# knights-lab/UTree

Measured on NVIDIA B200. Metric: reads/sec (150bp, L2-scale CTR, RC); k-mer lookups/sec in lookups_per_s, higher is better.
Workload: dtype u64

## Files before the change

utree_b200/csrc/kernels.cu:

```cuda
#include <cuda_runtime.h>
#include <stdint.h>
#include <stdio.h>
#include <stdlib.h>
#include <string.h>
#include "utb_internal.h"

#define SUFMASK 0xFFFFFFFFFFull
#define HIT_MISS 0xFFFFFFFFu
#define HIT_NOWIN 0xFFFFFFFEu

#define CK(call)                                                                 \
    do {                                                                         \
        cudaError_t e_ = (call);                                                 \
        if (e_ != cudaSuccess) {                                                 \
            utb_set_error("CUDA error %s at %s:%d (%s)", cudaGetErrorName(e_),   \
                          __FILE__, __LINE__, cudaGetErrorString(e_));           \
            return UTB_ERR_CUDA;                                                 \
        }                                                                        \
    } while (0)

struct DevDB {
    const uint32_t *binix32;
    const uint64_t *binix64;
    const uint8_t *recs;
// ... 26 lines not shown
    int sm_count;
    size_t nb_binix, nb_recs, nb_blob, nb_lab, nb_ktab, nb_sieve;
    int l2_window;
    size_t l2_window_bytes;
    float l2_hit_ratio;
};

__device__ __forceinline__ uint32_t classify4(uint32_t w, uint32_t &badbits) {
    const uint32_t u = w | 0x20202020u;
    const uint32_t code = ((u >> 1) ^ (u >> 2)) & 0x03030303u;
    const uint32_t c0 = code & 0x01010101u, c1 = (code >> 1) & 0x01010101u;
    const uint32_t both = c0 & c1;
    const uint32_t expect = 0x61616161u + (((c0 | c1) << 1) | ((c1 & ~c0) << 2)) + both * 0x11u;
    const uint32_t x = u ^ expect;
    const uint32_t inval = ((((x & 0x7F7F7F7Fu) + 0x7F7F7F7Fu) | x) >> 7) & 0x01010101u;
    badbits = (inval * 0x01020408u) >> 24;
    return code;
}

__device__ __forceinline__ uint64_t revcomp_word(uint64_t w) {
    uint64_t x = __brevll(~w);
    return ((x >> 1) & 0x5555555555555555ull) | ((x & 0x5555555555555555ull) << 1);
}
__device__ __forceinline__ uint64_t word_to_planes(uint64_t w) {
    uint64_t t;
    t = (w ^ (w >> 1)) & 0x2222222222222222ull; w ^= t ^ (t << 1);
    t = (w ^ (w >> 2)) & 0x0C0C0C0C0C0C0C0Cull; w ^= t ^ (t << 2);
    t = (w ^ (w >> 4)) & 0x00F000F000F000F0ull; w ^= t ^ (t << 4);
    t = (w ^ (w >> 8)) & 0x0000FF000000FF00ull; w ^= t ^ (t << 8);
    t = (w ^ (w >> 16)) & 0x00000000FFFF0000ull; w ^= t ^ (t << 16);
    return w;
}
__device__ __forceinline__ uint64_t planes_to_word(uint64_t w) {
    uint64_t t;
    t = (w ^ (w >> 16)) & 0x00000000FFFF0000ull; w ^= t ^ (t << 16);
    t = (w ^ (w >> 8)) & 0x0000FF000000FF00ull; w ^= t ^ (t << 8);
    t = (w ^ (w >> 4)) & 0x00F000F000F000F0ull; w ^= t ^ (t << 4);
    t = (w ^ (w >> 2)) & 0x0C0C0C0C0C0C0C0Cull; w ^= t ^ (t << 2);
    t = (w ^ (w >> 1)) & 0x2222222222222222ull; w ^= t ^ (t << 1);
    return w;
}
__device__ __forceinline__ uint32_t group_read(const uint32_t *__restrict__ grp_off, uint32_t n_reads, uint32_t g0, uint32_t lane) {
    uint32_t lo = 0, hi = n_reads;
    while (hi - lo > 1) {
        uint32_t mid = (lo + hi) >> 1;
        if (__ldg(grp_off + mid) <= g0) lo = mid; else hi = mid;
    }
    const uint32_t nb = lo + 1u + lane;
    const uint32_t bnd = nb < n_reads ? __ldg(grp_off + nb) : 0xFFFFFFFFu;
    const uint32_t starts = __reduce_or_sync(0xFFFFFFFFu, bnd - g0 < 32u ? 1u << (bnd - g0) : 0u);
    return lo + __popc(starts & (0xFFFFFFFFu >> (31u - lane)));
}
#define PK_GUARD 8u
template <bool WORDS, bool PLANES>
__global__ void __launch_bounds__(256)
pack_kernel(const uint8_t *__restrict__ raw, const uint64_t *__restrict__ seq_off,
            const uint32_t *__restrict__ seq_len, const uint32_t *__restrict__ grp_off,
            uint32_t n_reads, uint32_t n_groups, const uint32_t *__restrict__ dims,
            uint64_t *__restrict__ pk, uint32_t *__restrict__ bad, uint64_t *__restrict__ pl, uint32_t *__restrict__ rid) {
    if (dims) { n_reads = dims[0]; n_groups = dims[1]; }
    const uint32_t lane = threadIdx.x & 31u;
    for (uint64_t gw = ((uint64_t)blockIdx.x * blockDim.x + threadIdx.x) & ~31ull; gw < (uint64_t)n_groups + PK_GUARD; gw += (uint64_t)gridDim.x * blockDim.x) {
        const uint32_t g = (uint32_t)gw + lane;
        const uint32_t lo = (uint32_t)gw < n_groups ? group_read(grp_off, n_reads, (uint32_t)gw, lane) : 0u;
        if (g >= n_groups + PK_GUARD) continue;
        if (g >= n_groups) {
            if (WORDS) pk[g] = 0;
            if (PLANES) pl[g] = 0;
            bad[g] = 0xFFFFFFFFu;
            continue;
        }
        uint32_t k = g - __ldg(grp_off + lo);
        uint32_t len = __ldg(seq_len + lo);
        if (rid) rid[g] = lo;
        uint32_t b0 = k * 32u;
        uint32_t nv = len > b0 ? min(32u, len - b0) : 0u;
        uint64_t word = 0;
        uint32_t p1 = 0, p0 = 0;
        uint32_t badm = 0;
        if (nv) {
            uint64_t a = __ldg(seq_off + lo) + b0;
            const uint32_t *p = reinterpret_cast<const uint32_t *>(raw + (a & ~3ull));
            uint32_t sh = (uint32_t)(a & 3u) * 8u;
            uint32_t nw = (nv + 3u) >> 2;
            uint32_t prev = __ldg(p);
#pragma unroll
            for (uint32_t j = 0; j < 8; ++j) {
                uint32_t cur = (j < nw) ? __ldg(p + j + 1) : 0u;
                uint32_t w = __funnelshift_r(prev, cur, sh);
                prev = cur;
                uint32_t bb;
                const uint32_t code = classify4(w, bb);
                if (WORDS) word = (word << 8) | ((code * 0x40100401u) >> 24);
                if (PLANES) {
                    p1 = (p1 << 4) | ((((code >> 1) & 0x01010101u) * 0x08040201u) >> 24);
                    p0 = (p0 << 4) | (((code & 0x01010101u) * 0x08040201u) >> 24);
                }
                badm |= bb << (4u * j);
            }
        }
        if (nv < 32u) badm |= 0xFFFFFFFFu << nv;
        if (WORDS) pk[g] = word;
        if (PLANES) pl[g] = ((uint64_t)p1 << 32) | p0;
        bad[g] = badm;
    }
}

__device__ __forceinline__ bool window_at(const uint64_t *__restrict__ pk, const uint32_t *__restrict__ bad,
                                          uint32_t pos, uint64_t &w) {
    uint32_t g = pos >> 5, o = pos & 31u;
    uint64_t hi = pk[g], lo = pk[g + 1];
    uint32_t bh = bad[g], bl = bad[g + 1];
    uint32_t wb = o ? ((bh >> o) | (bl << (32u - o))) : bh;
    w = o ? ((hi << (2u * o)) | (lo >> (64u - 2u * o))) : hi;
    return wb == 0;
}


__device__ __forceinline__ uint64_t load_suffix(const uint8_t *__restrict__ recs, uint64_t byte_addr) {
    const uint32_t *p = reinterpret_cast<const uint32_t *>(recs + (byte_addr & ~3ull));
    uint32_t w0 = __ldg(p), w1 = __ldg(p + 1);
    uint32_t sh = (uint32_t)(byte_addr & 3u) * 8u;
    uint64_t v = ((uint64_t)w1 << 32) | w0;
    return (v >> sh) & SUFMASK;
}

__device__ __forceinline__ uint32_t load_ix(const DevDB &db, uint64_t rec) {
    const uint8_t *r = db.recs + rec * db.sz + 5;
    uint32_t v = (uint32_t)__ldg(r) | ((uint32_t)__ldg(r + 1) << 8);
    if (db.ix_bytes == 4) v |= ((uint32_t)__ldg(r + 2) << 16) | ((uint32_t)__ldg(r + 3) << 24);
    return v;
}

struct Probe {
    uint64_t pos, size, suf;
    bool live;
};

__device__ __forceinline__ void probe_begin(const DevDB &db, uint64_t word, Probe &q) {
    uint64_t p = word >> 40;
    uint64_t a, b;
    if (db.binix32) { a = __ldg(db.binix32 + p); b = __ldg(db.binix32 + p + 1); }
    else { a = __ldg(db.binix64 + p); b = __ldg(db.binix64 + p + 1); }
    q.suf = word & SUFMASK;
    q.live = a < b;
    if (b > db.num_nodes) q.live = false;
    q.pos = a;
    q.size = q.live ? b - a - 1 : 0;
}

template <int N>
__device__ __forceinline__ void probe_run(const DevDB &db, Probe (&q)[N]) {
    for (;;) {
        bool any = false;
#pragma unroll
        for (int i = 0; i < N; ++i) any |= q[i].size != 0;
// ... 223 lines not shown
    uint32_t r = HIT_NOWIN, ns = 0;
    if (valid) {
        if (NSTR == 2 && (slot & 1)) w = revcomp_word(w);
        if (TABLE) r = kt_lookup(db, w, &ns);
        else {
            Probe q[1];
            probe_begin(db, w, q[0]);
            probe_run<1>(db, q);
            r = probe_end(db, q[0]);
        }
    }
    if (pos < n_pos) hits[slot] = r;
    const uint32_t nv = __popc(__ballot_sync(0xFFFFFFFFu, valid));
    const uint32_t nh = __popc(__ballot_sync(0xFFFFFFFFu, r < HIT_NOWIN));
    for (int o = 16; o; o >>= 1) ns += __shfl_xor_sync(0xFFFFFFFFu, ns, o);
    if ((threadIdx.x & 31u) == 0) {
        const uint32_t c = blockIdx.x & (COUNTER_SLOTS - 1);
        if (nv) atomicAdd(counters + c, (unsigned long long)nv);
        if (nh) atomicAdd(counters + COUNTER_SLOTS + c, (unsigned long long)nh);
        if (ns) atomicAdd(counters + 3 * COUNTER_SLOTS + c, (unsigned long long)ns);
    }
}

#define Q_CHUNK 128u
#define Q_INVALID 0xFFFFFFFFu
struct WarpQueue {
    uint64_t base;
    uint32_t used;
    bool have;
};
__device__ __forceinline__ void wq_init(WarpQueue &q) { q.base = 0; q.used = Q_CHUNK; q.have = false; }
__device__ __forceinline__ void wq_retire(const WarpQueue &q, uint32_t lane, uint32_t *__restrict__ q_slots) {
    if (q.have) for (uint32_t j = q.used + lane; j < Q_CHUNK; j += 32) q_slots[q.base + j] = Q_INVALID;
}
__device__ __forceinline__ void wq_reserve(WarpQueue &q, uint32_t c, uint32_t lane, uint32_t *__restrict__ q_slots,
                                           unsigned long long *__restrict__ q_count, uint64_t q_cap) {
    if (q.used + c <= Q_CHUNK) return;
    wq_retire(q, lane, q_slots);
    unsigned long long nb = 0;
    if (lane == 0) nb = atomicAdd(q_count, (unsigned long long)Q_CHUNK);
    q.base = __shfl_sync(0xFFFFFFFFu, nb, 0);
    q.used = 0;
    q.have = q.base + Q_CHUNK <= q_cap;
}
struct HitSink {
    uint32_t *hits;
    uint32_t *hitmap;
    const uint32_t *rid, *grp_off;
    uint32_t *cnt;
    uint32_t sh;
};
__device__ __forceinline__ void sink_put(const HitSink &k, uint32_t slot, uint32_t r) {
    if (k.cnt) {
        const uint32_t rd = __ldg(k.rid + (slot >> k.sh));
        k.hits[((uint64_t)__ldg(k.grp_off + rd) << k.sh) + atomicAdd(k.cnt + rd, 1u)] = r;
    } else { k.hits[slot] = r; atomicOr(k.hitmap + (slot >> 5), 1u << (slot & 31u)); }
}
__device__ __noinline__ uint32_t resolve_inline(const DevDB &db, uint64_t x, uint32_t slot, const HitSink &sink) {
    const uint32_t r = kt_lookup(db, planes_to_word(x));
    if (r == HIT_MISS) return 0;
    sink_put(sink, slot, r);
    return 1;
}
template <int NSTR>
__device__ __forceinline__ uint32_t emit_survivors(const DevDB &db, WarpQueue &wq, uint32_t lane, bool passF, bool passR, uint64_t w, uint64_t rc,
                                                   uint32_t pos, uint64_t *__restrict__ q_words, uint32_t *__restrict__ q_slots,
                                                   unsigned long long *__restrict__ q_count, uint64_t q_cap, const HitSink &sink) {
    const uint32_t bF = __ballot_sync(0xFFFFFFFFu, passF);
    const uint32_t bR = NSTR == 2 ? __ballot_sync(0xFFFFFFFFu, passR) : 0u;
    const uint32_t cF = __popc(bF), c = cF + __popc(bR);
    uint32_t nh = 0;
    if (!c) return 0;
    wq_reserve(wq, c, lane, q_slots, q_count, q_cap);
    const uint32_t lt = (1u << lane) - 1u;
    if (wq.have) {
        const uint64_t at = wq.base + wq.used;
        if (passF) { const uint64_t i = at + __popc(bF & lt); q_words[i] = w; q_slots[i] = pos * NSTR; }
        if (passR) { const uint64_t i = at + cF + __popc(bR & lt); q_words[i] = rc; q_slots[i] = pos * NSTR + 1u; }
    } else {
        if (passF) nh += resolve_inline(db, w, pos * NSTR, sink);
        if (passR) nh += resolve_inline(db, rc, pos * NSTR + 1u, sink);
    }
    wq.used += c;
    return nh;
}

#define SV_DEAD 0xFFFFFFFFu
struct SvStep { uint32_t w1, w0, h, blk; };
__device__ __forceinline__ void sv_step(uint64_t cur, uint64_t next, uint32_t bh, uint32_t bl, uint32_t lane, SvStep &s) {
    s.w1 = __funnelshift_l((uint32_t)(next >> 32), (uint32_t)(cur >> 32), lane);
    s.w0 = __funnelshift_l((uint32_t)next, (uint32_t)cur, lane);
    const uint32_t m = sv_kmer16(s.w1, s.w0);
    s.h = sv_mhash(m, sv_rc16(m));
    s.blk = __funnelshift_r(bh, bl, lane) == 0u ? 0u : SV_DEAD;
}
template <int D, int SV_U>
__device__ __forceinline__ void sv_shifted(const uint32_t (&x)[SV_U + 1], uint32_t (&y)[SV_U + 1], uint32_t lane) {
    uint32_t rot[SV_U + 1];
#pragma unroll
    for (int u = 0; u <= SV_U; ++u) rot[u] = __shfl_sync(0xFFFFFFFFu, x[u], (lane + D) & 31u);
    const bool same = lane + D < 32u;
#pragma unroll
    for (int u = 0; u < SV_U; ++u) y[u] = same ? rot[u] : rot[u + 1];
    y[SV_U] = rot[SV_U];
}
__device__ __forceinline__ void sv_prefetch(const void *p) { asm volatile("prefetch.global.L1 [%0];" ::"l"(p)); }
template <int NSTR, int SV_U, int SV_MINB>
__global__ void __launch_bounds__(256, SV_MINB)
sieve_kernel(DevDB db, const uint64_t *__restrict__ pl, const uint32_t *__restrict__ bad, uint32_t n_pos,
             const uint32_t *__restrict__ n_groups_dev, unsigned long long *__restrict__ counters,
             uint64_t *__restrict__ q_words, uint32_t *__restrict__ q_slots, unsigned long long *__restrict__ q_count,
             uint64_t q_cap, const HitSink sink) {
    if (n_groups_dev) n_pos = *n_groups_dev * 32u;
    const uint32_t lane = threadIdx.x & 31u;
    const uint32_t n_steps = n_pos >> 5;
    const uint32_t n_warps = gridDim.x * (blockDim.x >> 5), wid = blockIdx.x * (blockDim.x >> 5) + (threadIdx.x >> 5);
    uint32_t per = (n_steps + n_warps - 1) / n_warps;
    per = (per + SV_U - 1) / SV_U * SV_U;
    const uint64_t s0 = (uint64_t)wid * per;
    const uint32_t s1 = s0 + per < n_steps ? (uint32_t)(s0 + per) : n_steps;
    const uint2 *__restrict__ sieve = db.sieve;
    const uint32_t n_lines = db.sv_lines;
    WarpQueue wq;
    wq_init(wq);
    uint32_t nv = 0, nh = 0;
    if (s0 < s1) {
        SvStep st[SV_U + 1];
        uint64_t cur = __ldg(pl + s0), next = __ldg(pl + s0 + 1);
        uint32_t bh = __ldg(bad + s0), bl = __ldg(bad + s0 + 1);
        sv_step(cur, next, bh, bl, lane, st[0]);
        for (uint32_t s = (uint32_t)s0; s < s1; s += SV_U) {
            {
                const uint32_t pf = s + 32u < n_steps ? s + 32u : n_steps;
                sv_prefetch(pl + pf); sv_prefetch(bad + pf);
            }
#pragma unroll
            for (int u = 1; u <= SV_U; ++u) {
                cur = next; bh = bl;
                next = __ldg(pl + s + u + 1); bl = __ldg(bad + s + u + 1);
                sv_step(cur, next, bh, bl, lane, st[u]);
            }
            uint32_t x[SV_U + 1], y1[SV_U + 1], y2[SV_U + 1];
#pragma unroll
            for (int u = 0; u <= SV_U; ++u) x[u] = st[u].h;
            sv_shifted<16, SV_U>(x, y1, lane);
#pragma unroll
            for (int u = 0; u < SV_U; ++u) st[u].blk |= sv_block(x[u], y1[u]);
            sv_shifted<1, SV_U>(x, y1, lane); sv_shifted<2, SV_U>(x, y2, lane);
#pragma unroll
            for (int u = 0; u <= SV_U; ++u) x[u] = __vimin3_u32(x[u], y1[u], y2[u]);
            sv_shifted<3, SV_U>(x, y1, lane); sv_shifted<6, SV_U>(x, y2, lane);
#pragma unroll
            for (int u = 0; u <= SV_U; ++u) x[u] = __vimin3_u32(x[u], y1[u], y2[u]);
            sv_shifted<8, SV_U>(x, y1, lane);
#pragma unroll
            for (int u = 0; u < SV_U; ++u) x[u] = x[u] < y1[u] ? x[u] : y1[u];
            uint2 v[SV_U];
#pragma unroll
            for (int u = 0; u < SV_U; ++u) {
                v[u] = make_uint2(0, 0);
                if (st[u].blk != SV_DEAD) v[u] = __ldg(sieve + ((sv_line(x[u], n_lines) << 4) | st[u].blk));
            }
#pragma unroll
            for (int u = 0; u < SV_U; ++u) {
                const bool live = st[u].blk != SV_DEAD;
                if (__any_sync(0xFFFFFFFFu, live)) {
                    const uint32_t r1 = ~__brev(st[u].w1), r0 = ~__brev(st[u].w0);
                    const bool tF = sv_test(v[u], st[u].w1, st[u].w0), tR = NSTR == 2 && sv_test(v[u], r1, r0);
                    nh += emit_survivors<NSTR>(db, wq, lane, live & tF, live & tR, ((uint64_t)st[u].w1 << 32) | st[u].w0, ((uint64_t)r1 << 32) | r0,
                                               (s + u) * 32u + lane, q_words, q_slots, q_count, q_cap, sink);
                    nv += live ? NSTR : 0;
                }
            }
            st[0] = st[SV_U];
        }
    }
    wq_retire(wq, lane, q_slots);
    for (int o = 16; o; o >>= 1) { nv += __shfl_xor_sync(0xFFFFFFFFu, nv, o); nh += __shfl_xor_sync(0xFFFFFFFFu, nh, o); }
    if (lane == 0) {
        const uint32_t cs = (blockIdx.x * 8 + (threadIdx.x >> 5)) & (COUNTER_SLOTS - 1);
        if (nv) atomicAdd(counters + cs, (unsigned long long)nv);
        if (nh) atomicAdd(counters + COUNTER_SLOTS + cs, (unsigned long long)nh);
    }
}

template <bool LISTS>
__global__ void __launch_bounds__(256, 6)
queue_lookup_kernel(DevDB db, const uint64_t *__restrict__ q_words, const uint32_t *__restrict__ q_slots,
                    const unsigned long long *__restrict__ q_count, uint64_t q_cap,
                    const HitSink sink, unsigned long long *__restrict__ counters) {
    const uint64_t n = *q_count < q_cap ? *q_count : q_cap;
    const uint64_t stride = (uint64_t)gridDim.x * blockDim.x;
// ... 1559 lines not shown
    memset(vs, 0, sizeof *vs);
}
static int vs_alloc(const utb_db *db, size_t max_bytes, vote_scratch *vs) {
    memset(vs, 0, sizeof *vs);
    const size_t nl = db->d.max_ix ? db->d.max_ix : 1;
    vs->n_cta = (unsigned)db->sm_count * VB_PER_SM;
    size_t pool = ((size_t)384 << 20) / (12 * nl);
    if (pool > VBIG_POOL_MAX) pool = VBIG_POOL_MAX;
    if (pool < 1) pool = 1;
    vs->vl.pool = (uint32_t)pool;
    vs->vl.split_slots = (size_t)128 << 10;
    (void)max_bytes;
    const char *e = getenv("UTB_VOTE_SPLIT_SLOTS");
    if (e && atoll(e) > 0) vs->vl.split_slots = (unsigned long long)atoll(e);
    vs->vl.sort_max = VB_SORT_MAX;
    e = getenv("UTB_VOTE_SORT_MAX");
    if (e && atoi(e) >= 0 && (uint32_t)atoi(e) < VB_SORT_MAX) vs->vl.sort_max = (uint32_t)atoi(e);
    cudaError_t err = cudaMalloc(&vs->vl.hist, (size_t)vs->n_cta * nl * 4);
    if (err == cudaSuccess) err = cudaMalloc(&vs->vl.tlab, (size_t)vs->n_cta * nl * 4);
    if (err == cudaSuccess) err = cudaMalloc(&vs->vl.tcnt, (size_t)vs->n_cta * nl * 4);
    if (err == cudaSuccess) err = cudaMalloc(&vs->vl.big_hist, pool * nl * 4);
    if (err == cudaSuccess) err = cudaMalloc(&vs->vl.big_tlab, pool * nl * 4);
    if (err == cudaSuccess) err = cudaMalloc(&vs->vl.big_tcnt, pool * nl * 4);
    if (err == cudaSuccess) err = cudaMalloc(&vs->vl.big_list, pool * 4);
    if (err == cudaSuccess) err = cudaMalloc(&vs->vl.big_state, (1 + 2 * pool) * 4);
    if (err == cudaSuccess) err = cudaMalloc(&vs->vl.work, 4);
    if (err == cudaSuccess) err = cudaMemset(vs->vl.hist, 0, (size_t)vs->n_cta * nl * 4);
    if (err == cudaSuccess) err = cudaMemset(vs->vl.big_hist, 0, pool * nl * 4);
    if (err != cudaSuccess) { vs_free(vs); CK(err); }
    return UTB_OK;
}
static int launch_long_vote(const utb_db *db, const VoteIn &in, utb_result *results, const uint32_t *gen_list, const uint32_t *gen_count,
                            vote_scratch *vs, unsigned long long *counters, cudaStream_t st) {
    CK(cudaMemsetAsync(vs->vl.big_state, 0, (1 + 2 * (size_t)vs->vl.pool) * 4, st));
    CK(cudaMemsetAsync(vs->vl.work, 0, 4, st));
    vote_block_kernel<<<vs->n_cta, VB_THREADS, 0, st>>>(db->d, in, results, gen_list, gen_count, vs->vl, counters);
    vote_big_count_kernel<<<(unsigned)db->sm_count * 4, VB_THREADS, 0, st>>>(db->d, in, vs->vl);
    vote_big_finish_kernel<<<vs->vl.pool < (uint32_t)db->sm_count ? vs->vl.pool : (unsigned)db->sm_count, VB_THREADS, 0, st>>>(db->d, vs->vl, results, counters);
    CK(cudaGetLastError());
    return UTB_OK;
}


struct utb_batch {
    utb_db *db;
    cudaStream_t st;
    cudaEvent_t done, ev[7];
    size_t max_bytes, max_reads;
    uint64_t max_groups;
    char *h_bytes; uint64_t *h_seq_off; uint32_t *h_seq_len; uint32_t *h_grp_off;
    utb_result *h_results; unsigned long long *h_counters;
    uint32_t *h_name_off, *h_name_len; char *h_text; uint32_t *h_text_len; size_t text_cap, h_text_cap;
    uint8_t *d_raw; uint64_t *d_seq_off; uint32_t *d_seq_len; uint32_t *d_grp_off;
    uint64_t *d_pk; uint32_t *d_bad; uint32_t *d_hits; uint64_t *d_pl;
    utb_result *d_results; uint32_t *d_gen_list; uint32_t *d_gen_count; uint32_t *d_warp_list; uint32_t *d_warp_count;
    uint32_t *d_name_off, *d_name_len, *d_line_len, *d_line_off, *d_scan_sums, *d_text_len; char *d_text;
    utb_batch_out out;
    unsigned long long *d_counters;
    vote_scratch vs;
    uint32_t *d_sel_cnt, *d_sel_off, *d_sel, *d_sel_gap, *d_sel_total, *h_sel_cnt, *h_sel, *h_sel_total; size_t sel_cap;
    uint64_t *d_qwords; uint32_t *d_qslots; unsigned long long *d_qcount; uint64_t q_cap;
    uint32_t *d_hitmap;
    uint32_t *d_rid, *d_hcnt;
    size_t n_reads; uint32_t n_groups; int do_rc; int in_flight; int used_sieve, used_lists;
    uint64_t launches;
    uint32_t *d_nl, *d_blk, *d_frame_err, *h_frame_err; int framed_on_device;
    uint32_t *d_frame_info;
    uint32_t *d_dims, *h_dims; const uint32_t *dims_dev;
    size_t nl_cap;
    int fastq; uint32_t min_qual;
    uint64_t *h_qual_off, *d_qual_off;
    int wrapped; const uint8_t *d_pack;
    char *h_join; uint8_t *d_join;
    uint32_t *d_wt, *d_wsums, *d_wtotal; uint64_t *d_kmask; size_t wt_cap;
};

extern "C" uint64_t utb_read_slots(uint32_t len) { return ((uint64_t)len + 1 + 31) / 32; }
extern "C" uint64_t utb_batch_max_slots(const utb_batch *b) { return b->max_groups; }
extern "C" char *utb_batch_bytes(utb_batch *b) { return b->h_bytes; }
extern "C" uint64_t *utb_batch_seq_off(utb_batch *b) { return b->h_seq_off; }
extern "C" uint32_t *utb_batch_seq_len(utb_batch *b) { return b->h_seq_len; }
extern "C" size_t utb_batch_max_bytes(const utb_batch *b) { return b->max_bytes; }
extern "C" size_t utb_batch_max_reads(const utb_batch *b) { return b->max_reads; }

extern "C" void utb_batch_destroy(utb_batch *b) {
    if (!b) return;
    cudaSetDevice(b->db->device);
    if (b->st) cudaStreamSynchronize(b->st);
    cudaFreeHost(b->h_bytes); cudaFreeHost(b->h_seq_off); cudaFreeHost(b->h_seq_len); cudaFreeHost(b->h_grp_off);
    cudaFreeHost(b->h_results); cudaFreeHost(b->h_counters);
    cudaFreeHost(b->h_name_off); cudaFreeHost(b->h_name_len); cudaFreeHost(b->h_text); cudaFreeHost(b->h_text_len);
    cudaFree(b->d_name_off); cudaFree(b->d_name_len); cudaFree(b->d_line_len); cudaFree(b->d_line_off); cudaFree(b->d_scan_sums);
    cudaFree(b->d_text_len); cudaFree(b->d_text);
    cudaFree(b->d_raw); cudaFree(b->d_seq_off); cudaFree(b->d_seq_len); cudaFree(b->d_grp_off);
    cudaFree(b->d_pk); cudaFree(b->d_bad); cudaFree(b->d_hits); cudaFree(b->d_results); cudaFree(b->d_pl);
    cudaFree(b->d_gen_list); cudaFree(b->d_gen_count); cudaFree(b->d_warp_list); cudaFree(b->d_warp_count); cudaFree(b->d_counters);
    vs_free(&b->vs);
    cudaFree(b->d_sel_cnt); cudaFree(b->d_sel_off); cudaFree(b->d_sel); cudaFree(b->d_sel_gap); cudaFree(b->d_sel_total);
    cudaFreeHost(b->h_sel_cnt); cudaFreeHost(b->h_sel); cudaFreeHost(b->h_sel_total);
    cudaFree(b->d_qwords); cudaFree(b->d_qslots); cudaFree(b->d_qcount); cudaFree(b->d_hitmap); cudaFree(b->d_rid); cudaFree(b->d_hcnt);
    cudaFree(b->d_nl); cudaFree(b->d_blk); cudaFree(b->d_frame_err); cudaFreeHost(b->h_frame_err);
    cudaFree(b->d_frame_info); cudaFree(b->d_dims); cudaFreeHost(b->h_dims);
    cudaFreeHost(b->h_qual_off); cudaFree(b->d_qual_off);
    cudaFreeHost(b->h_join); cudaFree(b->d_join); cudaFree(b->d_wt); cudaFree(b->d_wsums); cudaFree(b->d_wtotal); cudaFree(b->d_kmask);
    if (b->done) cudaEventDestroy(b->done);
    for (int i = 0; i < 7; ++i) if (b->ev[i]) cudaEventDestroy(b->ev[i]);
    if (b->st) cudaStreamDestroy(b->st);
    free(b);
}

extern "C" int utb_batch_create(utb_db *db, size_t max_bytes, size_t max_reads, utb_batch **out) {
    if (!db || !out || !max_bytes || !max_reads) { utb_set_error("utb_batch_create: bad argument"); return UTB_ERR_ARG; }
    *out = nullptr;
    if (max_bytes + 32 * max_reads >= ((uint64_t)1 << 32) - 4096) {
        utb_set_error("batch too large: positions must fit 32 bits"); return UTB_ERR_LIMIT;
    }
    CK(cudaSetDevice(db->device));
    utb_batch *b = (utb_batch *)calloc(1, sizeof(utb_batch));
    if (!b) { utb_set_error("out of memory"); return UTB_ERR_NOMEM; }
    b->db = db; b->max_bytes = max_bytes; b->max_reads = max_reads;
    b->max_groups = max_bytes / 32 + max_reads + 1;
    size_t npos = (size_t)b->max_groups * 32;
#define BK(call) do { cudaError_t e_ = (call); if (e_ != cudaSuccess) { utb_set_error("CUDA error %s at %s:%d (%s)", cudaGetErrorName(e_), __FILE__, __LINE__, cudaGetErrorString(e_)); utb_batch_destroy(b); return UTB_ERR_CUDA; } } while (0)
    BK(cudaStreamCreateWithFlags(&b->st, cudaStreamNonBlocking));
    BK(cudaEventCreateWithFlags(&b->done, cudaEventDisableTiming));
    for (int i = 0; i < 7; ++i) BK(cudaEventCreate(&b->ev[i]));
    BK(cudaMallocHost(&b->h_bytes, max_bytes + 64));
    BK(cudaMallocHost(&b->h_seq_off, max_reads * 8));
    BK(cudaMallocHost(&b->h_seq_len, max_reads * 4));
    BK(cudaMallocHost(&b->h_grp_off, (max_reads + 1) * 4));
    BK(cudaMallocHost(&b->h_results, max_reads * sizeof(utb_result)));
    BK(cudaMallocHost(&b->h_counters, 4 * COUNTER_SLOTS * 8));
    BK(cudaMallocHost(&b->h_name_off, (max_reads + 1) * 4));
    BK(cudaMallocHost(&b->h_name_len, (max_reads + 1) * 4));
    BK(cudaMallocHost(&b->h_text_len, 4));
    BK(cudaMalloc(&b->d_name_off, (max_reads + 1) * 4));
    BK(cudaMalloc(&b->d_name_len, (max_reads + 1) * 4));
    BK(cudaMalloc(&b->d_line_len, (max_reads + 1) * 4));
    BK(cudaMalloc(&b->d_line_off, (max_reads + 1) * 4));
    BK(cudaMalloc(&b->d_scan_sums, (max_reads / SCAN_TILE + 2) * 4));
    BK(cudaMalloc(&b->d_text_len, 4));
    BK(cudaMalloc(&b->d_dims, 8));
    BK(cudaMallocHost(&b->h_dims, 8));
    BK(cudaMalloc(&b->d_raw, max_bytes + 128));
    BK(cudaMalloc(&b->d_seq_off, max_reads * 8));
    BK(cudaMalloc(&b->d_seq_len, max_reads * 4));
    BK(cudaMalloc(&b->d_grp_off, (max_reads + 1) * 4));
    BK(cudaMalloc(&b->d_pk, (b->max_groups + PK_GUARD + 2) * 8));
    BK(cudaMalloc(&b->d_bad, (b->max_groups + PK_GUARD + 2) * 4));
    BK(cudaMalloc(&b->d_hits, npos * 2 * 4));
    BK(cudaMalloc(&b->d_results, max_reads * sizeof(utb_result)));
    BK(cudaMalloc(&b->d_gen_list, max_reads * 4));
    BK(cudaMalloc(&b->d_gen_count, 4));
    BK(cudaMalloc(&b->d_warp_list, max_reads * 4));
    BK(cudaMalloc(&b->d_warp_count, 4));
    BK(cudaMalloc(&b->d_counters, 4 * COUNTER_SLOTS * 8));
    if (vs_alloc(db, max_bytes, &b->vs)) { utb_batch_destroy(b); return UTB_ERR_CUDA; }
    BK(cudaMemset(b->d_raw, 0, max_bytes + 128));
    b->d_pack = b->d_raw;
    if (db->sieve) {
        b->q_cap = npos * 2 / 4 + 4096;
        const char *qc = getenv("UTB_QCAP");
        if (qc && atoll(qc) > 0) b->q_cap = (uint64_t)atoll(qc);
        b->q_cap = (b->q_cap + Q_CHUNK - 1) / Q_CHUNK * Q_CHUNK;
        BK(cudaMalloc(&b->d_qwords, b->q_cap * 8));
        BK(cudaMalloc(&b->d_qslots, b->q_cap * 4));
        BK(cudaMemset(b->d_qslots, 0xFF, b->q_cap * 4));
        BK(cudaMalloc(&b->d_qcount, 8));
        BK(cudaMalloc(&b->d_hitmap, (npos * 2 / 32 + 8) * 4));
        BK(cudaMalloc(&b->d_pl, (b->max_groups + PK_GUARD + 2) * 8));
        BK(cudaMalloc(&b->d_rid, (b->max_groups + PK_GUARD + 2) * 4));
        BK(cudaMalloc(&b->d_hcnt, (max_reads + 1) * 4));
    }
    if (db->l2_window) {
        cudaStreamAttrValue a;
        memset(&a, 0, sizeof a);
        a.accessPolicyWindow.base_ptr = db->binix;
        a.accessPolicyWindow.num_bytes = db->l2_window_bytes;
        a.accessPolicyWindow.hitRatio = db->l2_hit_ratio;
        a.accessPolicyWindow.hitProp = cudaAccessPropertyPersisting;
        a.accessPolicyWindow.missProp = cudaAccessPropertyStreaming;
        if (cudaStreamSetAttribute(b->st, cudaStreamAttributeAccessPolicyWindow, &a) != cudaSuccess) cudaGetLastError();
    }
#undef BK
    *out = b;
    return UTB_OK;
}

static unsigned gs_grid(const utb_batch *b, uint64_t n, uint32_t per, unsigned waves) {
    const uint64_t need = (n + per - 1) / per, cap = (uint64_t)b->db->sm_count * waves;
    return (unsigned)(need < cap ? (need ? need : 1) : cap);
}

static int launch_stages(utb_batch *b, bool timed) {
    const DevDB &d = b->db->d;
    const uint32_t n_reads = (uint32_t)b->n_reads, n_groups = b->n_groups;
    const uint32_t n_pos = n_groups * 32u;
    const uint32_t nstr = b->do_rc ? 2u : 1u;
    CK(cudaMemsetAsync(b->d_gen_count, 0, 4, b->st));
    CK(cudaMemsetAsync(b->d_counters, 0, 4 * COUNTER_SLOTS * 8, b->st));
    const bool sieve = b->db->sieve && (b->db->sieve_mode == 1 || (b->db->sieve_mode == 2 && b->db->ema_hit_rate < 0.40));
    const bool two_phase = b->db->use_table && sieve;
    if (timed) CK(cudaEventRecord(b->ev[0], b->st));
    if (n_reads) {
        const unsigned grid = gs_grid(b, (uint64_t)n_groups + PK_GUARD, 256, 32);
        if (!two_phase) pack_kernel<true, false><<<grid, 256, 0, b->st>>>(b->d_pack, b->d_seq_off, b->d_seq_len, b->d_grp_off,
                                                                        n_reads, n_groups, b->dims_dev, b->d_pk, b->d_bad, nullptr, b->d_rid);
        else if (b->out == UTB_OUT_SELECTIONS) pack_kernel<true, true><<<grid, 256, 0, b->st>>>(b->d_pack, b->d_seq_off, b->d_seq_len, b->d_grp_off,
                                                                        n_reads, n_groups, b->dims_dev, b->d_pk, b->d_bad, b->d_pl, b->d_rid);
        else pack_kernel<false, true><<<grid, 256, 0, b->st>>>(b->d_pack, b->d_seq_off, b->d_seq_len, b->d_grp_off,
                                                             n_reads, n_groups, b->dims_dev, nullptr, b->d_bad, b->d_pl, b->d_rid);
        b->launches++;
    }
    if (timed) CK(cudaEventRecord(b->ev[1], b->st));
    if (n_pos) {
        const unsigned nb = (unsigned)(((uint64_t)n_pos * nstr + 255) / 256);
        const unsigned sms = (unsigned)b->db->sm_count;
        b->used_sieve = sieve; b->used_lists = 0;
        if (two_phase) {
            CK(cudaMemsetAsync(b->d_qcount, 0, 8, b->st));
            HitSink sink;
            sink.hits = b->d_hits; sink.sh = nstr == 2 ? 6u : 5u;
            const bool lists = b->out != UTB_OUT_SELECTIONS;
            if (lists) { sink.hitmap = nullptr; sink.rid = b->d_rid; sink.grp_off = b->d_grp_off; sink.cnt = b->d_hcnt;
                         CK(cudaMemsetAsync(b->d_hcnt, 0, ((size_t)n_reads + 1) * 4, b->st)); }
            else { sink.hitmap = b->d_hitmap; sink.rid = nullptr; sink.grp_off = nullptr; sink.cnt = nullptr;
                   CK(cudaMemsetAsync(b->d_hitmap, 0, ((size_t)n_pos * nstr / 32 + 4) * 4, b->st)); }
            b->used_lists = lists;
            if (timed) CK(cudaEventRecord(b->ev[4], b->st));
            constexpr unsigned U = 6, MINB = 3;
            const unsigned wb = (n_groups + 8u * U - 1) / (8u * U);
            const unsigned pb = wb < sms * MINB ? (wb ? wb : 1u) : sms * MINB;
            const uint32_t *sv_groups = b->dims_dev ? b->dims_dev + 1 : nullptr;
            if (nstr == 2) sieve_kernel<2, U, MINB><<<pb, 256, 0, b->st>>>(d, b->d_pl, b->d_bad, n_pos, sv_groups, b->d_counters, b->d_qwords, b->d_qslots, b->d_qcount, b->q_cap, sink);
            else sieve_kernel<1, U, MINB><<<pb, 256, 0, b->st>>>(d, b->d_pl, b->d_bad, n_pos, sv_groups, b->d_counters, b->d_qwords, b->d_qslots, b->d_qcount, b->q_cap, sink);
            if (timed) CK(cudaEventRecord(b->ev[5], b->st));
            if (lists) queue_lookup_kernel<true><<<sms * 6, 256, 0, b->st>>>(d, b->d_qwords, b->d_qslots, b->d_qcount, b->q_cap, sink, b->d_counters);
            else queue_lookup_kernel<false><<<sms * 6, 256, 0, b->st>>>(d, b->d_qwords, b->d_qslots, b->d_qcount, b->q_cap, sink, b->d_counters);
            b->launches++;
        } else if (b->db->use_table) {
            if (nstr == 2) lookup_kernel<2, true><<<nb, 256, 0, b->st>>>(d, b->d_pk, b->d_bad, n_pos, b->dims_dev ? b->dims_dev + 1 : nullptr, b->d_hits, b->d_counters);
            else lookup_kernel<1, true><<<nb, 256, 0, b->st>>>(d, b->d_pk, b->d_bad, n_pos, b->dims_dev ? b->dims_dev + 1 : nullptr, b->d_hits, b->d_counters);
        } else {
            if (nstr == 2) lookup_kernel<2, false><<<nb, 256, 0, b->st>>>(d, b->d_pk, b->d_bad, n_pos, b->dims_dev ? b->dims_dev + 1 : nullptr, b->d_hits, b->d_counters);
            else lookup_kernel<1, false><<<nb, 256, 0, b->st>>>(d, b->d_pk, b->d_bad, n_pos, b->dims_dev ? b->dims_dev + 1 : nullptr, b->d_hits, b->d_counters);
        }
        b->launches++;
    }
    if (timed) CK(cudaEventRecord(b->ev[2], b->st));
    if (n_reads && b->out == UTB_OUT_SELECTIONS) {
        VoteIn in;
        in.hits = b->d_hits; in.grp_off = b->d_grp_off; in.seq_len = b->d_seq_len; in.off = nullptr; in.nstr = nstr;
        in.hitmap = b->used_sieve ? b->d_hitmap : nullptr;
        const uint32_t nt = (n_reads + SCAN_TILE - 1) / SCAN_TILE;
        shallow_select_kernel<<<gs_grid(b, n_reads, 128, 32), 128, 0, b->st>>>(d, in, b->d_pk, b->d_bad, n_reads, b->dims_dev, b->d_sel_cnt, b->d_sel_gap);
        scan_sums_kernel<false><<<gs_grid(b, nt, 1, 8), 256, 0, b->st>>>(b->d_sel_cnt, n_reads, b->dims_dev, nt, b->d_scan_sums);
        scan_top_kernel<false><<<1, 1024, 0, b->st>>>(b->d_scan_sums, nt, b->d_sel_total);
        scan_apply_kernel<false><<<gs_grid(b, nt, 1, 8), 256, 0, b->st>>>(b->d_sel_cnt, n_reads, b->dims_dev, nt, b->d_scan_sums, b->d_sel_off);
        shallow_compact_kernel<<<gs_grid(b, n_reads, 128, 32), 128, 0, b->st>>>(in, n_reads, b->dims_dev, b->d_sel_cnt, b->d_sel_off, b->d_sel_gap, b->d_sel);
        b->launches += 5;
    } else if (n_reads) {
        VoteIn in;
        in.hits = b->d_hits; in.grp_off = b->d_grp_off; in.seq_len = b->d_seq_len; in.off = nullptr; in.nstr = nstr;
        in.cnt = b->used_lists ? b->d_hcnt : nullptr;
        if (in.cnt) {
            CK(cudaMemsetAsync(b->d_warp_count, 0, 4, b->st));
            vote_thread_kernel<<<gs_grid(b, n_reads, VT_THREADS, 32), VT_THREADS, 0, b->st>>>(
                d, in, n_reads, b->dims_dev, b->d_results, b->d_warp_list, b->d_warp_count, b->d_counters);
            vote_warp_kernel<<<(unsigned)b->db->sm_count * 6, VW_WARPS * 32, 0, b->st>>>(
                d, in, n_reads, b->dims_dev, b->d_warp_list, b->d_warp_count, b->d_results, b->d_gen_list, b->d_gen_count, b->d_counters);
            b->launches++;
        } else
            vote_warp_kernel<<<gs_grid(b, n_reads, VW_WARPS, 32), VW_WARPS * 32, 0, b->st>>>(
                d, in, n_reads, b->dims_dev, nullptr, nullptr, b->d_results, b->d_gen_list, b->d_gen_count, b->d_counters);
        int rv = launch_long_vote(b->db, in, b->d_results, b->d_gen_list, b->d_gen_count, &b->vs, b->d_counters, b->st);
        if (rv) return rv;
        b->launches += 4;
    }
    if (timed) CK(cudaEventRecord(b->ev[3], b->st));
    CK(cudaGetLastError());
    return UTB_OK;
}

static size_t text_bytes(size_t max_bytes, size_t max_reads, size_t max_label) {
    return max_bytes + max_reads * (max_label + 48) + 64;
}
#define TEXT_LIMIT (((size_t)1 << 32) - 1)
extern "C" size_t utb_text_max_reads(size_t max_bytes, size_t max_reads, size_t max_label) {
// ... 402 lines not shown
extern "C" int utb_batch_rerun_device(utb_batch *b, int iters, float ms[4], uint64_t *launches) {
    if (!b || iters < 1) { utb_set_error("utb_batch_rerun_device: bad argument"); return UTB_ERR_ARG; }
    CK(cudaSetDevice(b->db->device));
    CK(cudaStreamSynchronize(b->st));
    float acc[4] = {0, 0, 0, 0};
    uint64_t l0 = b->launches;
    for (int it = 0; it < iters; ++it) {
        int rc = launch_stages(b, true);
        if (rc) return rc;
        CK(cudaMemcpyAsync(b->h_counters, b->d_counters, 4 * COUNTER_SLOTS * 8, cudaMemcpyDeviceToHost, b->st));
        CK(cudaStreamSynchronize(b->st));
        float t[4];
        rc = utb_batch_last_ms(b, t);
        if (rc) return rc;
        for (int i = 0; i < 4; ++i) acc[i] += t[i];
    }
    if (ms) for (int i = 0; i < 4; ++i) ms[i] = acc[i];
    if (launches) *launches = b->launches - l0;
    return UTB_OK;
}

extern "C" int utb_lookup_words(utb_db *db, const uint64_t *words, size_t n, uint32_t *ix) {
    if (!db || (!words && n) || (!ix && n)) { utb_set_error("utb_lookup_words: null argument"); return UTB_ERR_ARG; }
    if (!n) return UTB_OK;
    CK(cudaSetDevice(db->device));
    uint64_t *dw = nullptr; uint32_t *di = nullptr;
    CK(cudaMalloc(&dw, n * 8));
    CK(cudaMalloc(&di, n * 4));
    CK(cudaMemcpy(dw, words, n * 8, cudaMemcpyHostToDevice));
    if (db->use_table) lookup_words_kernel<true><<<(unsigned)((n + 255) / 256), 256>>>(db->d, dw, n, di);
    else lookup_words_kernel<false><<<(unsigned)((n + 255) / 256), 256>>>(db->d, dw, n, di);
    CK(cudaGetLastError());
    CK(cudaMemcpy(ix, di, n * 4, cudaMemcpyDeviceToHost));
    cudaFree(dw); cudaFree(di);
    return UTB_OK;
}

extern "C" int utb_pack_sequence(utb_db *db, const char *seq, uint32_t len, uint64_t *fwd, uint64_t *rc, uint8_t *valid) {
    if (!db || !seq || !fwd || !rc || !valid) { utb_set_error("utb_pack_sequence: null argument"); return UTB_ERR_ARG; }
    if (len > UTB_MAXSEQ) { utb_set_error("sequence too long"); return UTB_ERR_LIMIT; }
    if (!len) return UTB_OK;
    CK(cudaSetDevice(db->device));
    uint32_t n_groups = (uint32_t)utb_read_slots(len), n_pos = n_groups * 32;
    uint8_t *d_raw; uint64_t *d_off, *d_pk, *d_f, *d_r; uint32_t *d_len, *d_grp, *d_bad; uint8_t *d_v;
    CK(cudaMalloc(&d_raw, (size_t)len + 128)); CK(cudaMemset(d_raw, 0, (size_t)len + 128));
    CK(cudaMalloc(&d_off, 8)); CK(cudaMalloc(&d_len, 4)); CK(cudaMalloc(&d_grp, 8));
    CK(cudaMalloc(&d_pk, (size_t)(n_groups + PK_GUARD + 2) * 8)); CK(cudaMalloc(&d_bad, (size_t)(n_groups + PK_GUARD + 2) * 4));
    CK(cudaMalloc(&d_f, (size_t)n_pos * 8)); CK(cudaMalloc(&d_r, (size_t)n_pos * 8)); CK(cudaMalloc(&d_v, n_pos));
    uint64_t off = 1; uint32_t grp[2] = {0, n_groups};
    CK(cudaMemcpy(d_raw + 1, seq, len, cudaMemcpyHostToDevice));
    CK(cudaMemcpy(d_off, &off, 8, cudaMemcpyHostToDevice));
    CK(cudaMemcpy(d_len, &len, 4, cudaMemcpyHostToDevice));
    CK(cudaMemcpy(d_grp, grp, 8, cudaMemcpyHostToDevice));
    pack_kernel<true, false><<<(n_groups + PK_GUARD + 255) / 256, 256>>>(d_raw, d_off, d_len, d_grp, 1, n_groups, nullptr, d_pk, d_bad, nullptr, nullptr);
    expand_windows_kernel<<<(n_pos + 255) / 256, 256>>>(d_pk, d_bad, n_pos, d_f, d_r, d_v);
    CK(cudaGetLastError());
    CK(cudaMemcpy(fwd, d_f, (size_t)len * 8, cudaMemcpyDeviceToHost));
    CK(cudaMemcpy(rc, d_r, (size_t)len * 8, cudaMemcpyDeviceToHost));
    CK(cudaMemcpy(valid, d_v, len, cudaMemcpyDeviceToHost));
    cudaFree(d_raw); cudaFree(d_off); cudaFree(d_len); cudaFree(d_grp); cudaFree(d_pk); cudaFree(d_bad);
    cudaFree(d_f); cudaFree(d_r); cudaFree(d_v);
    return UTB_OK;
}

extern "C" int utb_vote_hits(utb_db *db, const uint32_t *hits, const uint64_t *off, size_t n_reads, utb_result *results) {
    if (!db || !off || !results || (!hits && n_reads && off[n_reads])) { utb_set_error("utb_vote_hits: null argument"); return UTB_ERR_ARG; }
    if (!n_reads) return UTB_OK;
    CK(cudaSetDevice(db->device));
    size_t nh = off[n_reads];
    uint32_t *d_hits, *d_gl, *d_gc; uint64_t *d_off; utb_result *d_res; unsigned long long *d_cnt; vote_scratch vs;
    CK(cudaMalloc(&d_hits, (nh + 1) * 4)); CK(cudaMalloc(&d_off, (n_reads + 1) * 8));
    CK(cudaMalloc(&d_res, n_reads * sizeof(utb_result)));
    CK(cudaMalloc(&d_gl, n_reads * 4)); CK(cudaMalloc(&d_gc, 4)); CK(cudaMalloc(&d_cnt, 4 * COUNTER_SLOTS * 8));
    { int rv = vs_alloc(db, (size_t)nh / 2 + 1, &vs); if (rv) return rv; }
    CK(cudaMemset(d_gc, 0, 4)); CK(cudaMemset(d_cnt, 0, 4 * COUNTER_SLOTS * 8));
    if (nh) CK(cudaMemcpy(d_hits, hits, nh * 4, cudaMemcpyHostToDevice));
    CK(cudaMemcpy(d_off, off, (n_reads + 1) * 8, cudaMemcpyHostToDevice));
    VoteIn in; in.hits = d_hits; in.grp_off = nullptr; in.seq_len = nullptr; in.off = d_off; in.nstr = 1; in.hitmap = nullptr;
    vote_warp_kernel<<<(unsigned)((n_reads + VW_WARPS - 1) / VW_WARPS), VW_WARPS * 32>>>(db->d, in, (uint32_t)n_reads, nullptr, nullptr, nullptr, d_res, d_gl, d_gc, d_cnt);
    { int rv = launch_long_vote(db, in, d_res, d_gl, d_gc, &vs, d_cnt, 0); if (rv) return rv; }
    CK(cudaMemcpy(results, d_res, n_reads * sizeof(utb_result), cudaMemcpyDeviceToHost));
    cudaFree(d_hits); cudaFree(d_off); cudaFree(d_res); cudaFree(d_gl); cudaFree(d_gc); cudaFree(d_cnt);
    vs_free(&vs);
    return UTB_OK;
}

extern "C" int utb_vote_hits_sparse(utb_db *db, const uint32_t *hits, const uint64_t *off, size_t n_reads, utb_result *results) {
    if (!db || !off || !results || (!hits && n_reads && off[n_reads])) { utb_set_error("utb_vote_hits_sparse: null argument"); return UTB_ERR_ARG; }
    if (!n_reads) return UTB_OK;
    CK(cudaSetDevice(db->device));
    uint64_t *poff = (uint64_t *)malloc((n_reads + 1) * 8);
    uint32_t *ph = (uint32_t *)malloc((off[n_reads] + 1) * 4);
    if (!poff || !ph) { free(poff); free(ph); utb_set_error("out of memory"); return UTB_ERR_NOMEM; }
    uint64_t tot = 0;
    for (size_t r = 0; r < n_reads; ++r) {
        poff[r] = tot;
        for (uint64_t i = off[r]; i < off[r + 1]; ++i) if (hits[i] < HIT_NOWIN) ph[tot++] = hits[i];
    }
    poff[n_reads] = tot;
    uint32_t *d_hits, *d_gl, *d_gc, *d_wl, *d_wc; uint64_t *d_off; utb_result *d_res; unsigned long long *d_cnt; vote_scratch vs;
    CK(cudaMalloc(&d_hits, (tot + 1) * 4)); CK(cudaMalloc(&d_off, (n_reads + 1) * 8));
    CK(cudaMalloc(&d_res, n_reads * sizeof(utb_result)));
    CK(cudaMalloc(&d_gl, n_reads * 4)); CK(cudaMalloc(&d_gc, 4)); CK(cudaMalloc(&d_wl, n_reads * 4)); CK(cudaMalloc(&d_wc, 4));
    CK(cudaMalloc(&d_cnt, 4 * COUNTER_SLOTS * 8));
    { int rv = vs_alloc(db, (size_t)tot / 2 + 1, &vs); if (rv) return rv; }
    CK(cudaMemset(d_gc, 0, 4)); CK(cudaMemset(d_wc, 0, 4)); CK(cudaMemset(d_cnt, 0, 4 * COUNTER_SLOTS * 8));
    if (tot) CK(cudaMemcpy(d_hits, ph, tot * 4, cudaMemcpyHostToDevice));
// ... 44 lines not shown
```

Measured before the change: 763.1 million.

## Fuse base-plane packing into sieve kernel, reading raw bytes directly

The sieve kernel now reads raw sequence bytes itself, classifies them with a shared-memory lookup table and builds the two bit planes and bad mask with warp ballots. This removes the separate plane output of the pack kernel, and pack is skipped entirely in two-phase mode unless selections are requested. The sieve also walks reads incrementally and writes the read-id map that pack used to produce. This removes a kernel launch and a round trip through global memory for the planes, at the cost of more per-step work and byte-granular loads inside the sieve.

```diff
diff --git a/utree_b200/csrc/kernels.cu b/utree_b200/csrc/kernels.cu
--- a/utree_b200/csrc/kernels.cu
+++ b/utree_b200/csrc/kernels.cu
@@ -102,12 +102,11 @@
     return lo + __popc(starts & (0xFFFFFFFFu >> (31u - lane)));
 }
 #define PK_GUARD 8u
-template <bool WORDS, bool PLANES>
 __global__ void __launch_bounds__(256)
 pack_kernel(const uint8_t *__restrict__ raw, const uint64_t *__restrict__ seq_off,
             const uint32_t *__restrict__ seq_len, const uint32_t *__restrict__ grp_off,
             uint32_t n_reads, uint32_t n_groups, const uint32_t *__restrict__ dims,
-            uint64_t *__restrict__ pk, uint32_t *__restrict__ bad, uint64_t *__restrict__ pl, uint32_t *__restrict__ rid) {
+            uint64_t *__restrict__ pk, uint32_t *__restrict__ bad, uint32_t *__restrict__ rid) {
     if (dims) { n_reads = dims[0]; n_groups = dims[1]; }
     const uint32_t lane = threadIdx.x & 31u;
     for (uint64_t gw = ((uint64_t)blockIdx.x * blockDim.x + threadIdx.x) & ~31ull; gw < (uint64_t)n_groups + PK_GUARD; gw += (uint64_t)gridDim.x * blockDim.x) {
@@ -115,8 +114,7 @@
         const uint32_t lo = (uint32_t)gw < n_groups ? group_read(grp_off, n_reads, (uint32_t)gw, lane) : 0u;
         if (g >= n_groups + PK_GUARD) continue;
         if (g >= n_groups) {
-            if (WORDS) pk[g] = 0;
-            if (PLANES) pl[g] = 0;
+            pk[g] = 0;
             bad[g] = 0xFFFFFFFFu;
             continue;
         }
@@ -126,7 +124,6 @@
         uint32_t b0 = k * 32u;
         uint32_t nv = len > b0 ? min(32u, len - b0) : 0u;
         uint64_t word = 0;
-        uint32_t p1 = 0, p0 = 0;
         uint32_t badm = 0;
         if (nv) {
             uint64_t a = __ldg(seq_off + lo) + b0;
@@ -141,17 +138,12 @@
                 prev = cur;
                 uint32_t bb;
                 const uint32_t code = classify4(w, bb);
-                if (WORDS) word = (word << 8) | ((code * 0x40100401u) >> 24);
-                if (PLANES) {
-                    p1 = (p1 << 4) | ((((code >> 1) & 0x01010101u) * 0x08040201u) >> 24);
-                    p0 = (p0 << 4) | (((code & 0x01010101u) * 0x08040201u) >> 24);
-                }
+                word = (word << 8) | ((code * 0x40100401u) >> 24);
                 badm |= bb << (4u * j);
             }
         }
         if (nv < 32u) badm |= 0xFFFFFFFFu << nv;
-        if (WORDS) pk[g] = word;
-        if (PLANES) pl[g] = ((uint64_t)p1 << 32) | p0;
+        pk[g] = word;
         bad[g] = badm;
     }
 }
@@ -481,7 +473,7 @@
 };
 __device__ __forceinline__ void sink_put(const HitSink &k, uint32_t slot, uint32_t r) {
     if (k.cnt) {
-        const uint32_t rd = __ldg(k.rid + (slot >> k.sh));
+        const uint32_t rd = k.rid[slot >> k.sh];
         k.hits[((uint64_t)__ldg(k.grp_off + rd) << k.sh) + atomicAdd(k.cnt + rd, 1u)] = r;
     } else { k.hits[slot] = r; atomicOr(k.hitmap + (slot >> 5), 1u << (slot & 31u)); }
 }
@@ -516,12 +508,12 @@
 
 #define SV_DEAD 0xFFFFFFFFu
 struct SvStep { uint32_t w1, w0, h, blk; };
-__device__ __forceinline__ void sv_step(uint64_t cur, uint64_t next, uint32_t bh, uint32_t bl, uint32_t lane, SvStep &s) {
-    s.w1 = __funnelshift_l((uint32_t)(next >> 32), (uint32_t)(cur >> 32), lane);
-    s.w0 = __funnelshift_l((uint32_t)next, (uint32_t)cur, lane);
+__device__ __forceinline__ void sv_step(uint2 cur, uint2 next, uint32_t bh, uint32_t bl, uint32_t lane, SvStep &s) {
+    s.w1 = __funnelshift_l(next.x, cur.x, lane);
+    s.w0 = __funnelshift_l(next.y, cur.y, lane);
     const uint32_t m = sv_kmer16(s.w1, s.w0);
     s.h = sv_mhash(m, sv_rc16(m));
-    s.blk = __funnelshift_r(bh, bl, lane) == 0u ? 0u : SV_DEAD;
+    s.blk = __funnelshift_l(bl, bh, lane) == 0u ? 0u : SV_DEAD;
 }
 template <int D, int SV_U>
 __device__ __forceinline__ void sv_shifted(const uint32_t (&x)[SV_U + 1], uint32_t (&y)[SV_U + 1], uint32_t lane) {
@@ -534,15 +526,42 @@
     y[SV_U] = rot[SV_U];
 }
 __device__ __forceinline__ void sv_prefetch(const void *p) { asm volatile("prefetch.global.L1 [%0];" ::"l"(p)); }
+struct SvRead { uint32_t r, off; int rem; };
+__device__ __forceinline__ bool sv_advance(SvRead &q, const uint64_t *__restrict__ seq_off, const uint32_t *__restrict__ seq_len,
+                                           uint32_t n_reads) {
+    q.off += 32u; q.rem -= 32;
+    if (q.rem >= 0) return false;
+    if (++q.r < n_reads) { q.off = (uint32_t)__ldg(seq_off + q.r); q.rem = (int)__ldg(seq_len + q.r); }
+    else q.rem = -0x40000000;
+    return true;
+}
+__device__ __forceinline__ uint32_t sv_byte(const uint8_t *rawl, const SvRead &q, uint32_t lr) {
+    return (int)lr < q.rem ? (uint32_t)__ldg(rawl + q.off) : 0u;
+}
+__device__ __forceinline__ int8_t sv_cls_value(uint32_t byte) {
+    uint32_t bb;
+    const uint32_t code = classify4(byte, bb) & 3u;
+    return (bb & 1u) ? (int8_t)0 : (int8_t)("\xff\x01\x03\x02"[code]);
+}
+__device__ __forceinline__ uint2 sv_group(const int8_t *cls, uint32_t c, uint32_t &bad) {
+    const int v = cls[c];
+    bad = __ballot_sync(0xFFFFFFFFu, v == 0);
+    return make_uint2(__ballot_sync(0xFFFFFFFFu, v >= 2), __ballot_sync(0xFFFFFFFFu, (uint32_t)v < 3u));
+}
 template <int NSTR, int SV_U, int SV_MINB>
 __global__ void __launch_bounds__(256, SV_MINB)
-sieve_kernel(DevDB db, const uint64_t *__restrict__ pl, const uint32_t *__restrict__ bad, uint32_t n_pos,
-             const uint32_t *__restrict__ n_groups_dev, unsigned long long *__restrict__ counters,
+sieve_kernel(DevDB db, const uint8_t *__restrict__ raw, uint32_t raw_cap, const uint64_t *__restrict__ seq_off,
+             const uint32_t *__restrict__ seq_len, const uint32_t *__restrict__ grp_off, uint32_t n_reads, uint32_t n_groups,
+             const uint32_t *__restrict__ dims, uint32_t *__restrict__ rid, unsigned long long *__restrict__ counters,
              uint64_t *__restrict__ q_words, uint32_t *__restrict__ q_slots, unsigned long long *__restrict__ q_count,
              uint64_t q_cap, const HitSink sink) {
-    if (n_groups_dev) n_pos = *n_groups_dev * 32u;
-    const uint32_t lane = threadIdx.x & 31u;
-    const uint32_t n_steps = n_pos >> 5;
+    __shared__ int8_t cls[256];
+    for (uint32_t i = threadIdx.x; i < 256u; i += blockDim.x) cls[i] = sv_cls_value(i);
+    __syncthreads();
+    if (dims) { n_reads = dims[0]; n_groups = dims[1]; }
+    const uint32_t lane = threadIdx.x & 31u, lr = 31u - lane;
+    const uint8_t *rawl = raw + lr;
+    const uint32_t n_steps = n_groups;
     const uint32_t n_warps = gridDim.x * (blockDim.x >> 5), wid = blockIdx.x * (blockDim.x >> 5) + (threadIdx.x >> 5);
     uint32_t per = (n_steps + n_warps - 1) / n_warps;
     per = (per + SV_U - 1) / SV_U * SV_U;
@@ -554,19 +573,43 @@
     wq_init(wq);
     uint32_t nv = 0, nh = 0;
     if (s0 < s1) {
+        SvRead q;
+        {
+            uint32_t lo = 0, hi = n_reads;
+            while (hi - lo > 1) {
+                const uint32_t mid = (lo + hi) >> 1;
+                if (__ldg(grp_off + mid) <= (uint32_t)s0) lo = mid; else hi = mid;
+            }
+            const uint32_t k = (uint32_t)s0 - __ldg(grp_off + lo);
+            q.r = lo; q.off = (uint32_t)__ldg(seq_off + lo) + 32u * k; q.rem = (int)__ldg(seq_len + lo) - (int)(32u * k);
+        }
+        if (lane == 0) rid[s0] = q.r;
         SvStep st[SV_U + 1];
-        uint64_t cur = __ldg(pl + s0), next = __ldg(pl + s0 + 1);
-        uint32_t bh = __ldg(bad + s0), bl = __ldg(bad + s0 + 1);
-        sv_step(cur, next, bh, bl, lane, st[0]);
+        uint32_t bh, bl;
+        const uint2 first = sv_group(cls, sv_byte(rawl, q, lr), bh);
+        sv_advance(q, seq_off, seq_len, n_reads);
+        if (lane == 0 && s0 + 1u < s1) rid[s0 + 1u] = q.r;
+        uint2 next = sv_group(cls, sv_byte(rawl, q, lr), bl);
+        sv_step(first, next, bh, bl, lane, st[0]);
         for (uint32_t s = (uint32_t)s0; s < s1; s += SV_U) {
             {
-                const uint32_t pf = s + 32u < n_steps ? s + 32u : n_steps;
-                sv_prefetch(pl + pf); sv_prefetch(bad + pf);
+                const uint32_t rp = min(q.r + 32u, n_reads - 1u);
+                sv_prefetch(raw + min(q.off + 512u, raw_cap)); sv_prefetch(seq_off + rp); sv_prefetch(seq_len + rp);
             }
+            const uint32_t r_t = q.r;
+            uint32_t c[SV_U], cross = 0;
+#pragma unroll
+            for (int u = 0; u < SV_U; ++u) {
+                if (sv_advance(q, seq_off, seq_len, n_reads)) cross |= 1u << u;
+                c[u] = sv_byte(rawl, q, lr);
+            }
+            if (lane < (uint32_t)SV_U && s + 2u + lane < s1) rid[s + 2u + lane] = r_t + __popc(cross & ((2u << lane) - 1u));
+            __syncwarp();
 #pragma unroll
             for (int u = 1; u <= SV_U; ++u) {
-                cur = next; bh = bl;
-                next = __ldg(pl + s + u + 1); bl = __ldg(bad + s + u + 1);
+                const uint2 cur = next;
+                bh = bl;
+                next = sv_group(cls, c[u - 1], bl);
                 sv_step(cur, next, bh, bl, lane, st[u]);
             }
             uint32_t x[SV_U + 1], y1[SV_U + 1], y2[SV_U + 1];
@@ -2232,7 +2275,7 @@
     utb_result *h_results; unsigned long long *h_counters;
     uint32_t *h_name_off, *h_name_len; char *h_text; uint32_t *h_text_len; size_t text_cap, h_text_cap;
     uint8_t *d_raw; uint64_t *d_seq_off; uint32_t *d_seq_len; uint32_t *d_grp_off;
-    uint64_t *d_pk; uint32_t *d_bad; uint32_t *d_hits; uint64_t *d_pl;
+    uint64_t *d_pk; uint32_t *d_bad; uint32_t *d_hits;
     utb_result *d_results; uint32_t *d_gen_list; uint32_t *d_gen_count; uint32_t *d_warp_list; uint32_t *d_warp_count;
     uint32_t *d_name_off, *d_name_len, *d_line_len, *d_line_off, *d_scan_sums, *d_text_len; char *d_text;
     utb_batch_out out;
@@ -2273,7 +2316,7 @@
     cudaFree(b->d_name_off); cudaFree(b->d_name_len); cudaFree(b->d_line_len); cudaFree(b->d_line_off); cudaFree(b->d_scan_sums);
     cudaFree(b->d_text_len); cudaFree(b->d_text);
     cudaFree(b->d_raw); cudaFree(b->d_seq_off); cudaFree(b->d_seq_len); cudaFree(b->d_grp_off);
-    cudaFree(b->d_pk); cudaFree(b->d_bad); cudaFree(b->d_hits); cudaFree(b->d_results); cudaFree(b->d_pl);
+    cudaFree(b->d_pk); cudaFree(b->d_bad); cudaFree(b->d_hits); cudaFree(b->d_results);
     cudaFree(b->d_gen_list); cudaFree(b->d_gen_count); cudaFree(b->d_warp_list); cudaFree(b->d_warp_count); cudaFree(b->d_counters);
     vs_free(&b->vs);
     cudaFree(b->d_sel_cnt); cudaFree(b->d_sel_off); cudaFree(b->d_sel); cudaFree(b->d_sel_gap); cudaFree(b->d_sel_total);
@@ -2348,7 +2391,6 @@
         BK(cudaMemset(b->d_qslots, 0xFF, b->q_cap * 4));
         BK(cudaMalloc(&b->d_qcount, 8));
         BK(cudaMalloc(&b->d_hitmap, (npos * 2 / 32 + 8) * 4));
-        BK(cudaMalloc(&b->d_pl, (b->max_groups + PK_GUARD + 2) * 8));
         BK(cudaMalloc(&b->d_rid, (b->max_groups + PK_GUARD + 2) * 4));
         BK(cudaMalloc(&b->d_hcnt, (max_reads + 1) * 4));
     }
@@ -2382,14 +2424,9 @@
     const bool sieve = b->db->sieve && (b->db->sieve_mode == 1 || (b->db->sieve_mode == 2 && b->db->ema_hit_rate < 0.40));
     const bool two_phase = b->db->use_table && sieve;
     if (timed) CK(cudaEventRecord(b->ev[0], b->st));
-    if (n_reads) {
-        const unsigned grid = gs_grid(b, (uint64_t)n_groups + PK_GUARD, 256, 32);
-        if (!two_phase) pack_kernel<true, false><<<grid, 256, 0, b->st>>>(b->d_pack, b->d_seq_off, b->d_seq_len, b->d_grp_off,
-                                                                        n_reads, n_groups, b->dims_dev, b->d_pk, b->d_bad, nullptr, b->d_rid);
-        else if (b->out == UTB_OUT_SELECTIONS) pack_kernel<true, true><<<grid, 256, 0, b->st>>>(b->d_pack, b->d_seq_off, b->d_seq_len, b->d_grp_off,
-                                                                        n_reads, n_groups, b->dims_dev, b->d_pk, b->d_bad, b->d_pl, b->d_rid);
-        else pack_kernel<false, true><<<grid, 256, 0, b->st>>>(b->d_pack, b->d_seq_off, b->d_seq_len, b->d_grp_off,
-                                                             n_reads, n_groups, b->dims_dev, nullptr, b->d_bad, b->d_pl, b->d_rid);
+    if (n_reads && (!two_phase || b->out == UTB_OUT_SELECTIONS)) {
+        pack_kernel<<<gs_grid(b, (uint64_t)n_groups + PK_GUARD, 256, 32), 256, 0, b->st>>>(b->d_pack, b->d_seq_off, b->d_seq_len, b->d_grp_off,
+                                                                                          n_reads, n_groups, b->dims_dev, b->d_pk, b->d_bad, b->d_rid);
         b->launches++;
     }
     if (timed) CK(cudaEventRecord(b->ev[1], b->st));
@@ -2411,9 +2448,11 @@
             constexpr unsigned U = 6, MINB = 3;
             const unsigned wb = (n_groups + 8u * U - 1) / (8u * U);
             const unsigned pb = wb < sms * MINB ? (wb ? wb : 1u) : sms * MINB;
-            const uint32_t *sv_groups = b->dims_dev ? b->dims_dev + 1 : nullptr;
-            if (nstr == 2) sieve_kernel<2, U, MINB><<<pb, 256, 0, b->st>>>(d, b->d_pl, b->d_bad, n_pos, sv_groups, b->d_counters, b->d_qwords, b->d_qslots, b->d_qcount, b->q_cap, sink);
-            else sieve_kernel<1, U, MINB><<<pb, 256, 0, b->st>>>(d, b->d_pl, b->d_bad, n_pos, sv_groups, b->d_counters, b->d_qwords, b->d_qslots, b->d_qcount, b->q_cap, sink);
+            const uint32_t raw_cap = (uint32_t)b->max_bytes;
+            if (nstr == 2) sieve_kernel<2, U, MINB><<<pb, 256, 0, b->st>>>(d, b->d_pack, raw_cap, b->d_seq_off, b->d_seq_len, b->d_grp_off, n_reads, n_groups, b->dims_dev,
+                                                                           b->d_rid, b->d_counters, b->d_qwords, b->d_qslots, b->d_qcount, b->q_cap, sink);
+            else sieve_kernel<1, U, MINB><<<pb, 256, 0, b->st>>>(d, b->d_pack, raw_cap, b->d_seq_off, b->d_seq_len, b->d_grp_off, n_reads, n_groups, b->dims_dev,
+                                                                 b->d_rid, b->d_counters, b->d_qwords, b->d_qslots, b->d_qcount, b->q_cap, sink);
             if (timed) CK(cudaEventRecord(b->ev[5], b->st));
             if (lists) queue_lookup_kernel<true><<<sms * 6, 256, 0, b->st>>>(d, b->d_qwords, b->d_qslots, b->d_qcount, b->q_cap, sink, b->d_counters);
             else queue_lookup_kernel<false><<<sms * 6, 256, 0, b->st>>>(d, b->d_qwords, b->d_qslots, b->d_qcount, b->q_cap, sink, b->d_counters);
@@ -2922,7 +2961,7 @@
     CK(cudaMemcpy(d_off, &off, 8, cudaMemcpyHostToDevice));
     CK(cudaMemcpy(d_len, &len, 4, cudaMemcpyHostToDevice));
     CK(cudaMemcpy(d_grp, grp, 8, cudaMemcpyHostToDevice));
-    pack_kernel<true, false><<<(n_groups + PK_GUARD + 255) / 256, 256>>>(d_raw, d_off, d_len, d_grp, 1, n_groups, nullptr, d_pk, d_bad, nullptr, nullptr);
+    pack_kernel<<<(n_groups + PK_GUARD + 255) / 256, 256>>>(d_raw, d_off, d_len, d_grp, 1, n_groups, nullptr, d_pk, d_bad, nullptr);
     expand_windows_kernel<<<(n_pos + 255) / 256, 256>>>(d_pk, d_bad, n_pos, d_f, d_r, d_v);
     CK(cudaGetLastError());
     CK(cudaMemcpy(fwd, d_f, (size_t)len * 8, cudaMemcpyDeviceToHost));
```

Result: no change. 760.9 million, median of 6 (-0.3%).
